# alibaba/euler

Hardware: AMD Instinct MI355X
Metric: sampled edges/sec (whole node), 2-hop fanout=[25,10], 100M-node power-law graph (higher is better)
Workload: dtype f64; 1 GPU; synthetic RMAT-marginal power-law graph, 100000000 nodes / 1000001082 edges (min degree 1), f32 weights uniform [0.5,8), weighted CDF-inversion SampleNeighbor, fanout [25,10], 131072 uniform-random roots per step per GPU, TF dense layout; graph_bytes_per_gpu=55296276736, partitioning=none, streams=3, repeats=1, full=False, ranks=1

## Files before the change

### euler_amd/_lib.py

```python
import ctypes as C
import os

HERE = os.path.dirname(os.path.abspath(__file__))
LIB_PATH = os.environ.get("EULER_GPU_LIB_PATH") or os.path.join(HERE, "lib", "libeuler_gpu.so")

OK, EINVAL, ENOMEM, EHIP, ENOGRAPH, EIO, EEMPTY = 0, -1, -2, -3, -4, -5, -6
LAYOUT_CORE, LAYOUT_TF = 0, 1
F32, BF16, F16 = 0, 1, 2

u64p = C.POINTER(C.c_uint64)
i64p = C.POINTER(C.c_int64)
i32p = C.POINTER(C.c_int32)
f32p = C.POINTER(C.c_float)
u8p = C.POINTER(C.c_uint8)
vp = C.c_void_p


class HostCSR(C.Structure):
    _fields_ = [("n_rows", C.c_int64), ("n_edge_types", C.c_int32),
                ("n_node_types", C.c_int32), ("row_id", u64p),
                ("row_ptr", i64p), ("type_end", i32p), ("nbr", u64p),
                ("prefix_w", f32p), ("type_prefix", f32p),
                ("node_type", i32p), ("node_weight", f32p),
                ("sampler_order", u64p),
# ... 70 lines not shown
    "euler_gpu_sample_graph_label": (C.c_int, [vp, vp, C.c_uint64, C.c_uint32, C.c_int32, vp]),
    "euler_gpu_get_graph_by_label": (C.c_int, [vp, vp, vp, C.c_int64, vp, i64p, vp]),
    "euler_gpu_whole_graph_block": (C.c_int, [vp, vp, vp, C.c_int64, i32p, C.c_int32, C.c_int32,
                                              C.c_int64, i64p, vp]),
    "euler_gpu_graph_destroy": (None, [vp]),
    "euler_gpu_graph_num_nodes": (C.c_int64, [vp]),
    "euler_gpu_graph_num_edges": (C.c_int64, [vp]),
    "euler_gpu_graph_num_edge_types": (C.c_int32, [vp]),
    "euler_gpu_graph_num_node_types": (C.c_int32, [vp]),
    "euler_gpu_graph_device": (C.c_int, [vp]),
    "euler_gpu_graph_bytes": (C.c_int64, [vp]),
    "euler_gpu_graph_node_weight_sums": (C.c_int, [vp, f32p]),
    "euler_gpu_graph_set_node_sampler": (C.c_int, [vp, C.c_int64, u64p, i32p, f32p, C.c_int32]),
    "euler_gpu_last_fanout_kernel": (C.c_char_p, []),
    "euler_gpu_graph_index_overflow_rows": (C.c_int, [vp, u64p, C.c_int64, i64p]),
    "euler_gpu_graph_export_rows": (C.c_int, [vp, u64p, C.c_int64, i64p, i32p, u64p,
                                              f32p, f32p]),
    "InitQueryProxy": (C.c_bool, [C.c_char_p]),
    "euler_gpu_default_graph": (vp, []),
    "euler_gpu_graph_partitions": (C.c_int32, [vp]),
    "euler_gpu_sample_neighbor": (C.c_int, [vp, vp, C.c_uint64, C.c_uint32, vp,
                                            C.c_int64, vp, C.c_int32, i32p, C.c_int32,
                                            C.c_int32, C.c_int32, C.c_int64, vp, vp,
                                            vp, vp]),
    "euler_gpu_sample_fanout_workspace": (C.c_size_t, [C.c_int64, i32p, C.c_int32]),
    "euler_gpu_sample_fanout": (C.c_int, [vp, vp, C.c_uint64, C.c_uint32, vp,
                                          C.c_int64, i32p, C.c_int32, i32p, C.c_int32,
                                          C.c_int64, C.POINTER(vp), C.POINTER(vp),
                                          C.POINTER(vp), vp]),
    "euler_gpu_sample_fanout_multi": (C.c_int, [vp, vp, C.c_uint64, C.c_uint32, C.c_uint32, vp,
# ... 257 lines not shown
```

### euler_amd/csrc/common.h

```cpp
#pragma once

#include <hip/hip_runtime.h>
#include <stdint.h>

#include <atomic>
#include <map>
#include <mutex>
#include <string>
#include <vector>

#include "../../include/euler_gpu.h"
#include "../../include/euler_gpu_measure.h"
#include "philox.h"

namespace euler_gpu {

void SetError(const std::string& msg);
int Fail(int code, const std::string& msg);

#define EG_HIP(expr)                                                        \
  do {                                                                      \
    hipError_t _e = (expr);                                                 \
    if (_e != hipSuccess)                                                   \
      return ::euler_gpu::Fail(EULER_GPU_EHIP,                              \
// ... 30 lines not shown
  const float* pivots;
  int64_t piv_off[kPivotLevels + 1];
  const float* bpiv;
  int64_t bpiv_off[kPivotLevels + 1];
  const struct EdgeBlock* blk;
  const float* skip1;
  int64_t n_blk;
  const struct WbRec* wrec;
  const struct EdgeBlock* wb;
  int64_t n_wb;
  const uint8_t* wbg;
  int32_t wbg_stride;
  const uint8_t* trec;
  int32_t trec_stride;
  const uint8_t* fat;
  int32_t wb_lean_ok;
};

inline bool HasBlockSearch(const GraphView& v) { return v.blk != nullptr || v.wbg != nullptr; }

constexpr int kEdgesPerBlock = 10;
struct alignas(128) EdgeBlock {
  float pw[kEdgesPerBlock];
  float prev_last;
  uint32_t pad;
  uint64_t nbr[kEdgesPerBlock];
};
static_assert(sizeof(EdgeBlock) == 128, "EdgeBlock must be one 128-byte line");

constexpr int kWavesPerSimd = 8;
// ... 84 lines not shown
  std::vector<std::pair<void*, int64_t>> edge_allocs;
  std::pair<void*, int64_t> edge_sampler_alloc{nullptr, 0};
  std::vector<int64_t> bin_host_ptr;
  std::vector<int32_t> bin_host_idx;
  std::vector<uint8_t> bin_host_val;
  int32_t bin_host_slots = 0;
  mutable std::mutex bin_mu;
  mutable euler_gpu::FeatTable node_bin{};
  mutable bool node_bin_ready = false;
  mutable std::mutex ws_mu;
  mutable std::recursive_mutex launch_mu;
  mutable std::map<void*, std::pair<void*, size_t>> ws;
  mutable std::map<void*, int> ws_parity;
  mutable std::atomic<void*> last_stream{nullptr};
  mutable std::atomic<int> wb_tried{0};
  std::vector<uint32_t> wb_overflow_rows;
  mutable std::atomic<int> blk_ready{0};
  struct FlowTableDense { void* p = nullptr; size_t rows = 0; uint32_t next_epoch = 1; };
  mutable std::map<void*, FlowTableDense> flow_tables;
  int32_t shards = 1;
  int32_t label_slot = -1;
  mutable std::mutex label_mu;
  mutable bool labels_ready = false;
  mutable int64_t n_labels = 0;
  mutable int64_t n_labelled = 0;
  mutable const uint64_t* label_nodes = nullptr;
  mutable const int64_t* label_start = nullptr;
  mutable std::vector<std::pair<void*, int64_t>> label_allocs;
  mutable std::vector<int64_t> label_off_host;
  mutable std::vector<uint8_t> label_bytes_host;
// ... 110 lines not shown
```

### euler_amd/csrc/fanout_local.h

```cpp
#ifndef EULER_AMD_CSRC_FANOUT_LOCAL_H_
#define EULER_AMD_CSRC_FANOUT_LOCAL_H_

#include <hip/hip_runtime.h>

#include "k1_search.h"
#include "wb_index.h"

namespace euler_gpu {

struct SmallDiv {
  uint32_t d, m;
  __host__ void Set(uint32_t div) { d = div; m = div <= 1 ? 0u : 0xFFFFFFFFu / div + 1u; }
  __device__ __forceinline__ uint32_t operator()(uint32_t n) const {
    return d <= 1 ? n : __umulhi(n, m);
  }
};

struct FanoutLocalArgs {
  GraphView g;
  uint64_t seed;
  const uint64_t* roots;
  int64_t n;
  int64_t default_node;
  uint32_t call_id;
// ... 510 lines not shown
  if (__ballot(cold0 || cold1) != 0ull) {
#pragma nounroll
    for (int s = 0; s < (TWO ? 2 : 1); ++s) {
      if (s == 0 ? cold0 : cold1) {
        const float* nw = g.prefix_w + rec.lo;
        const uint32_t mid = (uint32_t)RandomSelect(nw, 0, (uint64_t)(rec.deg - 1u), s == 0 ? u0 : u1);
        const uint64_t ci = g.nbr[rec.lo + mid];
        const float cw = __fsub_rn(nw[mid], mid == 0u ? 0.f : nw[mid - 1]);
        if (s == 0) { id[0] = ci; w[0] = cw; m[0] = rec.lo + mid; }
        else { id[1] = ci; w[1] = cw; m[1] = rec.lo + mid; }
      }
    }
  }
}

struct WbSeg {
  uint32_t wb_lo, row_deg;
  uint32_t lo, deg;
  float row_total, lim_b, lim_e;
  uint32_t row_lo;
};

__device__ __forceinline__ bool FatFind(const GraphView& g, const uint64_t id, uint4* hd, uint4* tl,
                                        const uint4** slot) {
  uint64_t h = Mix64(id) & g.hash_mask;
  for (uint64_t probes = 0; probes <= g.hash_mask; ++probes) {
    const uint4* s = reinterpret_cast<const uint4*>(g.fat + h * 64);
    const uint4 a = s[0], b = s[1];
    if ((int32_t)b.y == -1) return false;
    if (a.x == (uint32_t)id && a.y == (uint32_t)(id >> 32)) { *hd = a; *tl = b; *slot = s; return true; }
// ... 347 lines not shown
  L.o_mask = o; o += (uint32_t)gr * 8;
  L.o_sw = o; o += s * 4;
  L.o_w1 = o; o += p * 4;
  L.o_st = o; o += (uint32_t)cap * 4;
  L.o_slot = o; o += (p * 2 + 3) & ~3u;
  L.o_rvalid = o; o += ((uint32_t)gr + 3) & ~3u;
  L.o_t1 = o; L.o_t2 = o;
  if (typed) {
    o += (p + 3) & ~3u;
    L.o_t2 = o; o += (s + 3) & ~3u;
  }
  L.bytes = (o + 15) & ~15u;
  return L;
}

template <bool WIDE, int WPS, bool UNIFORM = false, int WB = 0>
__global__ __launch_bounds__(256, WPS) void SampleFanoutLeanKernel(
    const FanoutLocalArgs a) {
  extern __shared__ __align__(16) uint8_t fl_smem[];
  const int lane = threadIdx.x & 63;
  const int wave_in_block = __builtin_amdgcn_readfirstlane((int)(threadIdx.x >> 6));
  const int waves_per_block = blockDim.x >> 6;
  const FanoutLeanLds L = FanoutLeanLayout(a.gr, a.c1, a.c2, a.cap, WB >= 3 && WB <= 5);
  uint8_t* base = fl_smem + (size_t)wave_in_block * a.wave_lds;
  uint64_t* s_sid = reinterpret_cast<uint64_t*>(base + L.o_sid);
  uint64_t* s_c1 = reinterpret_cast<uint64_t*>(base + L.o_c1);
  uint64_t* s_slotid = reinterpret_cast<uint64_t*>(base + L.o_slotid);
  unsigned long long* s_mask = reinterpret_cast<unsigned long long*>(base + L.o_mask);
  float* s_sw = reinterpret_cast<float*>(base + L.o_sw);
  float* s_w1 = reinterpret_cast<float*>(base + L.o_w1);
  int32_t* s_st = reinterpret_cast<int32_t*>(base + L.o_st);
// ... 211 lines not shown
        const bool live = in && deg > 0 && !EG_FL_ABLATE(a, 2);
        uint64_t id[2]; float w[2]; uint32_t m[2];
        int32_t tt[2] = {a.t2, a.t2};
        bool sentinel = false;
        Philox4 pb;
        if (WB == 4 || WB == 5) WbSampleTypedPair4<WB == 5>(g, w4, a.type_mode, a.et2, a.k, a.seed, tile_call + 1u, node, xp, live,
                                        true, id, w, m, tt, &sentinel);
        else if (WB == 3) WbSampleTypedPair(g, wt, a.type_mode, a.et2, a.k, a.seed, tile_call + 1u, node, xp, live,
                                            true, id, w, m, tt, &sentinel);
        else pb = RngBlock(a.seed, tile_call + 1u, kDomainNeighbor, node, xp);
        if (WB >= 3 && WB <= 5) {}
        else if (WB == 6) UniformSamplePairG2(g, ws, ws, a.t2, a.t2, live, live, UnitFromWords(pb.w[0], pb.w[1]),
                                              UnitFromWords(pb.w[2], pb.w[3]), id, w, m);
        else if (WB == 2) WbSamplePairG(g, ws, a.t2, live, UnitFromWords(pb.w[0], pb.w[1]),
                                   UnitFromWords(pb.w[2], pb.w[3]), id, w, m);
        else if (WB) WbSamplePair(g, wr, live, UnitFromWords(pb.w[0], pb.w[1]),
                                  UnitFromWords(pb.w[2], pb.w[3]), id, w, m);
        else if (UNIFORM) LeanSamplePairUniform(g, lo, deg, total, live, UnitFromWords(pb.w[0], pb.w[1]),
                                           UnitFromWords(pb.w[2], pb.w[3]), id, w, m);
        else LeanSamplePair(g, lo, deg, total, live, UnitFromWords(pb.w[0], pb.w[1]),
                            UnitFromWords(pb.w[2], pb.w[3]), id, w, m, EG_FL_ABLATE_BITS(a));
        if (in) {
          fl_u64x2 iv;
          iv.x = live ? id[0] : (uint64_t)a.default_node;
          iv.y = live ? id[1] : (uint64_t)a.default_node;
          *reinterpret_cast<fl_u64x2*>(s_sid + sl * c2 + 2u * xp) = iv;
          *reinterpret_cast<float2*>(s_sw + sl * c2 + 2u * xp) =
              make_float2(live ? w[0] : 0.f, live ? w[1] : 0.f);
          if (xp == 0) s_st[sl] = live ? a.t2 : -1;
          if (WB >= 3 && WB <= 5) {
// ... 118 lines not shown
```

### euler_amd/csrc/fanout_plain.h

```cpp
#ifndef EULER_AMD_CSRC_FANOUT_PLAIN_H_
#define EULER_AMD_CSRC_FANOUT_PLAIN_H_

#include <hip/hip_runtime.h>

#include "fanout_local.h"

namespace euler_gpu {

struct FanoutPlainArgs {
  const WbRec* wrec;
  const EdgeBlock* wb;
  const float* prefix_w;
  const uint64_t* nbr;
  const uint64_t* roots;
  uint64_t* id1; float* w1; int32_t* ty1;
  uint64_t* id2; float* w2; int32_t* ty2;
  uint32_t* row_index;
  const uint32_t* call_ids;
  uint64_t seed, id_base, id_stride;
  int64_t n, n_rows, default_node, mb_n;
  uint32_t call_id, call_stride;
  int32_t c1, c2, gr, cap, wave_lds;
};

constexpr uint32_t kStageLines = 128;
constexpr uint32_t kStageBytes = kStageLines * 48 + kStageLines * 4;
// ... 247 lines not shown
__device__ __forceinline__ int64_t PlainFindRow(const FanoutPlainArgs& a, const uint64_t id) {
  const uint64_t d = id - a.id_base;
  if (id < a.id_base) return -1;
  if (a.id_stride == 1) return d < (uint64_t)a.n_rows ? (int64_t)d : -1;
  const uint64_t r = d / a.id_stride;
  return (r * a.id_stride == d && r < (uint64_t)a.n_rows) ? (int64_t)r : -1;
}

__device__ __forceinline__ WbRec PlainLoadRec(const FanoutPlainArgs& a, const uint64_t node) {
  WbRec wr{0u, 0u, 0u, 0.f};
  const int64_t row = PlainFindRow(a, node);
  if (row >= 0) wr = a.wrec[row];
  return wr;
}

template <int WPS, bool COOP, bool LITE2 = false>
__global__ __launch_bounds__(256, WPS) void SampleFanoutPlainKernel(const FanoutPlainArgs a) {
  extern __shared__ __align__(16) uint8_t fp_smem[];
  const uint32_t lane = threadIdx.x & 63u;
  const int wave_in_block = __builtin_amdgcn_readfirstlane((int)(threadIdx.x >> 6));
  const int waves_per_block = blockDim.x >> 6;
  const uint32_t c1 = (uint32_t)a.c1, c2 = (uint32_t)a.c2, gr = (uint32_t)a.gr, cap = (uint32_t)a.cap;
  const FanoutPlainLds L = FanoutPlainLayout(a.gr, a.c1, a.c2, a.cap, COOP);
  uint8_t* base = fp_smem + (size_t)wave_in_block * a.wave_lds;
  float4* s_stage = reinterpret_cast<float4*>(base + L.o_stage);
  uint32_t* s_blk = reinterpret_cast<uint32_t*>(base + L.o_blk);
  uint64_t* s_sid = reinterpret_cast<uint64_t*>(base + L.o_sid);
  uint64_t* s_c1 = reinterpret_cast<uint64_t*>(base + L.o_c1);
  unsigned long long* s_mask = reinterpret_cast<unsigned long long*>(base + L.o_mask);
  float* s_sw = reinterpret_cast<float*>(base + L.o_sw);
  float* s_w1 = reinterpret_cast<float*>(base + L.o_w1);
// ... 120 lines not shown
      const uint32_t rs = d_hp2(lane2), x2 = lane2 - __umul24(rs, hp2);
      const bool act2 = rs < RPI;
      for (uint32_t sb = 0; sb < ns; sb += RPI) {
        const uint32_t sl = sb + rs;
        const bool in = act2 && sl < ns;
        uint64_t child = 0;
        WbRec cr{0u, 0u, 0u, 0.f};
        if (in) { child = s_c1[s_rep[s0 + sl]]; cr = PlainLoadRec(a, child); }
        const bool lv = in && cr.deg > 0u;
        uint64_t i2[2]; float w2[2]; uint32_t m2[2];
        const Philox4 pb = RngBlock(a.seed, call + 1u, kDomainNeighbor, child, x2);
        if (COOP) {
          const uint32_t left = ns - sb < RPI ? ns - sb : RPI;
          WaveSamplePairs(a, lane, __umul24(left, hp2), s_stage, s_blk, cr, lv, lv, UnitFromWords(pb.w[0], pb.w[1]),
                          UnitFromWords(pb.w[2], pb.w[3]), i2, w2, m2);
        } else if (LITE2) {
          PlainSamplePairLite(a, cr, lv, lv, UnitFromWords(pb.w[0], pb.w[1]), UnitFromWords(pb.w[2], pb.w[3]), i2, w2);
        } else {
          PlainSamplePair(a, cr, lv, lv, UnitFromWords(pb.w[0], pb.w[1]), UnitFromWords(pb.w[2], pb.w[3]),
                          i2, w2, m2);
        }
        if (in) {
          fl_u64x2 iv;
          iv.x = lv ? i2[0] : (uint64_t)a.default_node;
          iv.y = lv ? i2[1] : (uint64_t)a.default_node;
          const uint32_t at = __umul24(sl, c2) + 2u * x2;
          *reinterpret_cast<fl_u64x2*>(s_sid + at) = iv;
          *reinterpret_cast<float2*>(s_sw + at) = make_float2(lv ? w2[0] : 0.f, lv ? w2[1] : 0.f);
          if (x2 == 0) s_st[sl] = lv ? 0 : -1;
        }
// ... 104 lines not shown
```

### euler_amd/csrc/graph_build.hip

```cpp
#include <hip/hip_runtime.h>
#include <sys/stat.h>
#include <hipcub/hipcub.hpp>

#include <algorithm>
#include <atomic>
#include <cstdlib>
#include <cmath>
#include <cstring>
#include <map>
#include <memory>
#include <mutex>
#include <sstream>

#include "device_fns.h"
#include "device_mem.h"
#include "wb_index.h"

namespace euler_gpu {


namespace {
thread_local std::string g_last_error;
std::mutex g_default_mu;
euler_gpu_graph* g_default_graph = nullptr;
}

void SetError(const std::string& msg) { g_last_error = msg; }
int Fail(int code, const std::string& msg) {
  g_last_error = msg;
  return code;
}
// ... 773 lines not shown
    }
    const RowMeta m = LoadRowMeta(g, lo);
    const uint32_t deg = (uint32_t)m.type_end[g.T - 1];
    EdgeBlock e;
    if (WbBuildBlock(g.prefix_w, g.nbr, (uint32_t)m.row_ptr, deg, g.prefix_w[m.row_ptr + deg - 1],
                     (uint32_t)(b - (int64_t)wb_lo[lo]), &e)) {
      ++mine;
      const unsigned long long k = atomicAdd(overflows + 1, 1ull);
      if (k < (unsigned long long)kWbOverflowKeep) ovf_rows[k] = (uint32_t)lo;
    }
    wb[b] = e;
  }
  if (mine != 0) atomicAdd(overflows, mine);
}

__global__ __launch_bounds__(256) void FatFillKernel(GraphView g, const uint8_t* trec, int32_t trec_stride,
                                                     uint8_t* fat) {
  const uint64_t stride = (uint64_t)gridDim.x * blockDim.x;
  for (uint64_t h = (uint64_t)blockIdx.x * blockDim.x + threadIdx.x; h <= g.hash_mask; h += stride) {
    const uint64_t key = g.hash_slots[2 * h];
    const int64_t row = (int64_t)g.hash_slots[2 * h + 1];
    uint4 a = make_uint4(0u, 0u, 0u, 0u), b = make_uint4(0u, 0xFFFFFFFFu, 0u, 0u), c = make_uint4(0u, 0u, 0u, 0u);
    if (row >= 0) {
      const uint8_t* rec = trec + row * (int64_t)trec_stride;
      const uint32_t* hd = reinterpret_cast<const uint32_t*>(rec);
      const int32_t* te = reinterpret_cast<const int32_t*>(rec + 8);
      const float* lim = reinterpret_cast<const float*>(rec + 8 + 4 * g.T);
      const RowMeta m = LoadRowMeta(g, row);
      const int32_t t1 = g.T - 1;
      a = make_uint4((uint32_t)key, (uint32_t)(key >> 32), hd[0], hd[1]);
// ... 41 lines not shown
    if (f >= 0 && f <= 1) ppm = (int64_t)(f * 1e6);
  }
  g_wb_budget_ppm.store(ppm);
  g_wb_budget_bytes.store(bytes);
}

bool WbFits(size_t need) {
  WbBudgetFromEnv();
  size_t free_b = 0, total_b = 0;
  if (hipMemGetInfo(&free_b, &total_b) != hipSuccess) { (void)hipGetLastError(); return false; }
  const int64_t cap = g_wb_budget_bytes.load();
  if (cap >= 0 && need > (size_t)cap) return false;
  const double frac = (double)g_wb_budget_ppm.load() * 1e-6;
  if ((double)need > frac * (double)free_b) return false;
  return need + ((size_t)1 << 30) <= free_b;
}

int BuildWbIndex(GraphBuilder* b) {
  GraphView& v = b->g->view;
  if (v.monotone != 0 && v.uniform_w != 0 && (v.T > 1 || v.map_mode != 0) && v.n_rows > 0 && v.n_edges > 0 &&
      v.n_edges < ((int64_t)1 << 31)) {
    const int32_t stride = v.T == 1 ? 16 : 8 + 12 * v.T;
    if (!WbFits((size_t)v.n_rows * stride)) return EULER_GPU_OK;
    uint8_t* trec = b->Alloc<uint8_t>((size_t)v.n_rows * stride + 16);
    if (b->rc != EULER_GPU_OK) return b->rc;
    hipLaunchKernelGGL(WbRecKernel, dim3((v.n_rows + 255) / 256), dim3(256), 0, 0, v, (const uint32_t*)nullptr,
                       trec, stride);
    EG_HIP(hipGetLastError());
    EG_HIP(hipDeviceSynchronize());
    v.trec = trec; v.trec_stride = stride;
// ... 39 lines not shown
  EG_HIP(hipMemset(ovf, 0, 16 + 4 * kWbOverflowKeep));
  if (n_wb > 0)
    hipLaunchKernelGGL(WbFillKernel, dim3(GridFor(n_wb, block)), dim3(block), 0, 0, v, wb_lo, n_wb, wb, ovf);
  EG_HIP(hipGetLastError());
  EG_HIP(hipDeviceSynchronize());
  unsigned long long n_ovf = 0;
  EG_HIP(hipMemcpy(&n_ovf, ovf, 8, hipMemcpyDeviceToHost));
  {
    const size_t keep = (size_t)std::min<unsigned long long>(n_ovf, (unsigned long long)kWbOverflowKeep);
    b->g->wb_overflow_rows.resize(keep);
    if (keep > 0) EG_HIP(hipMemcpy(b->g->wb_overflow_rows.data(), ovf + 2, keep * 4, hipMemcpyDeviceToHost));
  }
  v.wrec = rec; v.wb = wb; v.n_wb = n_wb; v.wbg = wbg; v.wbg_stride = stride;
  v.trec = wbg; v.trec_stride = stride;
  v.wb_lean_ok = (double)n_ovf <= 0.002 * (double)n_wb ? 1 : 0;
  return BuildFatSlots(b);
}

int EnsureWbIndex(const euler_gpu_graph* cg) {
  euler_gpu_graph* g = const_cast<euler_gpu_graph*>(cg);
  if (g->wb_tried.load(std::memory_order_acquire) != 0) return EULER_GPU_OK;
  std::lock_guard<std::mutex> lk(g_blocked_mu);
  if (g->wb_tried.load(std::memory_order_acquire) != 0) return EULER_GPU_OK;
  DeviceGuard dg(g->device);
  GraphBuilder b;
  b.g.reset(g);
  const int rc = BuildWbIndex(&b);
  if (rc == EULER_GPU_OK) b.Commit();
  b.g.release();
  if (rc != EULER_GPU_OK) {
    (void)hipGetLastError();
    (void)hipDeviceSynchronize();
    (void)hipGetLastError();
    b.Release();
    GraphView& v = g->view;
    v.wb = nullptr; v.wbg = nullptr; v.wrec = nullptr; v.n_wb = 0; v.wb_lean_ok = 0;
    v.trec = nullptr; v.trec_stride = 0; v.fat = nullptr;
  }
  g->wb_tried.store(1, std::memory_order_release);
  return EULER_GPU_OK;
}

std::atomic<int> g_blk_fail_next{0};

int EnsureBlockedIndex(const euler_gpu_graph* cg) {
  euler_gpu_graph* g = const_cast<euler_gpu_graph*>(cg);
  if (g->blk_ready.load(std::memory_order_acquire) != 0) return EULER_GPU_OK;
  std::lock_guard<std::mutex> lk(g_blocked_mu);
  if (g->blk_ready.load(std::memory_order_acquire) != 0) return EULER_GPU_OK;
  DeviceGuard dg(g->device);
  GraphBuilder b;
  b.g.reset(g);
// ... 235 lines not shown
int euler_gpu_graph_index_overflow_rows(const euler_gpu_graph* g, uint64_t* ids_host, int64_t cap,
                                        int64_t* n_host) {
  if (!g || !n_host || cap < 0 || (cap > 0 && !ids_host))
    return Fail(EULER_GPU_EINVAL, "index_overflow_rows: bad arguments");
  *n_host = 0;
  const int rc = EnsureWbIndex(g);
  if (rc != EULER_GPU_OK) return rc;
  const GraphView& v = g->view;
  if (v.map_mode != 0) return EULER_GPU_OK;
  int64_t n = 0;
  for (uint32_t row : g->wb_overflow_rows) {
    if (n >= cap) break;
    ids_host[n++] = v.id_base + v.id_stride * (uint64_t)row;
  }
  *n_host = n;
  return EULER_GPU_OK;
}

int euler_gpu_graph_node_weight_sums(const euler_gpu_graph* g, float* out_host) {
  if (!g || !out_host) return Fail(EULER_GPU_EINVAL, "node_weight_sums: null");
  for (size_t i = 0; i < g->node_weight_sums.size(); ++i)
    out_host[i] = g->node_weight_sums[i];
  return EULER_GPU_OK;
}

int euler_gpu_graph_export_rows(const euler_gpu_graph* g, const uint64_t* ids_host,
                                int64_t n, int64_t* row_ptr_host,
                                int32_t* type_end_host, uint64_t* nbr_host,
                                float* prefix_w_host, float* type_prefix_host) {
  if (!g) return Fail(EULER_GPU_ENOGRAPH, "export_rows: null graph");
// ... 104 lines not shown
```

### euler_amd/csrc/sample_kernels.hip

```cpp
#include <hip/hip_runtime.h>
#include <hipcub/hipcub.hpp>

#include <cmath>
#include <vector>

#include "device_mem.h"
#include "k1_args.h"
#include "k1_search.h"
#include "fanout_local.h"
#include "fanout_plain.h"

extern thread_local int g_feature_vec4;
namespace euler_gpu { extern thread_local int g_walk_collapse, g_walk_grid, g_walk_tail, g_walk_lean; extern std::atomic<int> g_walk_path_ch, g_n2v_list_big, g_n2v_list_big_parent, g_n2v_list_merged, g_n2v_walk_tickets; }
namespace euler_gpu { extern std::atomic<int> g_sharded_self_exchange, g_sharded_walk_enqueued, g_sharded_walk_tail, g_sharded_walk_split; }
namespace euler_gpu { extern std::atomic<int> g_flow_fused; extern std::atomic<int> g_flow_rowpos; }
namespace euler_gpu { extern std::atomic<int> g_blk_fail_next; }
namespace euler_gpu { extern thread_local int g_label_hash_bits; }
namespace euler_gpu { extern thread_local int g_root_host_batch, g_adj_scan, g_adj_long_row, g_sum_scalar; }

namespace euler_gpu {

struct DedupArgs {
  GraphView g;
  const uint64_t* roots;
// ... 445 lines not shown
thread_local int g_fanout_fused = 1;
thread_local int g_full_nb_balanced = 1;
thread_local int g_n2v_big = 8192;
thread_local int g_fanout_local = 1;
thread_local int g_fl_roots = 0;
thread_local int g_fl_cap = 0;
thread_local int g_fl_block = 0;
thread_local int g_fl_wide = 1;
thread_local int g_fl_grid_cap = -1;
thread_local int g_fl_min_roots = 32768;
thread_local int g_fl_plain = 2;
thread_local int g_fl_wps = 5;
thread_local int g_fp_on = 1;
thread_local int g_fp_coop = 0;
thread_local int g_fp_lite2 = 0;
thread_local int g_fp_wps = 5;
thread_local int g_fl_wb = 1;
thread_local int g_fl_typed_regs = 1;
thread_local int g_k1_sets_lds = 1;
thread_local int g_fl_fat = 1;
thread_local int g_blk_policy = 0;
thread_local int g_fl_ablate = 0;
thread_local int g_k1_typed_pivot = 1;
thread_local uint32_t* t_fl_row_index = nullptr;
thread_local int t_fl_took_lean = 0;
thread_local const char* t_fl_last_kernel = "";
thread_local void* g_fl_debug = nullptr;

int SamplingView(const euler_gpu_graph* g, GraphView* out) {
  const bool wb = g_fl_wb != 0 && g_k1_variant == 6;
  if (wb) {
    const int rc = EnsureWbIndex(g);
    if (rc != EULER_GPU_OK) return rc;
  }
  const bool wb_serves = wb && g->view.wbg != nullptr && (g->view.wb_lean_ok != 0 || g_blk_policy == 1);
  if (g_k1_variant == 6 && !wb_serves && g->blk_ready.load(std::memory_order_acquire) == 0) {
    const int rc = EnsureBlockedIndex(g);
    if (rc != EULER_GPU_OK) return rc;
  }
  *out = g->view;
  if (!wb) { out->wb = nullptr; out->wbg = nullptr; out->wrec = nullptr; out->n_wb = 0; out->wb_lean_ok = 0;
             out->trec = nullptr; out->trec_stride = 0; out->fat = nullptr; }
  if (g_fl_fat == 0) out->fat = nullptr;
  return EULER_GPU_OK;
}

template <bool TF_LAYOUT, int U, bool BLOCKED>
__device__ __forceinline__ void PivotPass(const SampleNbArgs& a, const int64_t n_roots,
                                          const int64_t stride_rows,
                                          const int32_t stride_slots) {
  const int64_t total = n_roots * (int64_t)a.count;
  const int64_t stride = (int64_t)gridDim.x * blockDim.x * U;
  int64_t s = ((int64_t)blockIdx.x * blockDim.x + threadIdx.x) * U;
  if (s >= total) return;
  int64_t r = s / a.count;
  int32_t j = (int32_t)(s - r * a.count);
  const int32_t t = a.et[0];
// ... 784 lines not shown
          ll = FanoutLeanLayout(gr, c1, c2, lcap, lean_t);
        }
        const bool use_wb0 = v.uniform_w == 0 && f.g.wrec != nullptr && f.g.wb != nullptr && v.wb_lean_ok != 0;
        if (g_fp_on != 0 && (t_concurrent != 1 || g_fp_on == 2 || big) && plain && !typed_hops && use_wb0 && f.wide) {
          int32_t pgr = g_fl_roots > 0 ? gr : 4;
          while (multi != nullptr && pgr > 1 && multi->n_per % pgr != 0) pgr >>= 1;
          int32_t pcap = g_fl_cap > 0 ? g_fl_cap : (g_fp_coop != 0 ? 64 / (c2 / 2 > 0 ? c2 / 2 : 1) : 32);
          if (pcap > pgr * c1) pcap = pgr * c1;
          const int pblock = (g_fl_block == 64 || g_fl_block == 128 || g_fl_block == 256) ? g_fl_block : 128;
          const bool coop = g_fp_coop != 0;
          const FanoutPlainLds pl = FanoutPlainLayout(pgr, c1, c2, pcap, coop);
          const int64_t tp = (int64_t)pgr * c1 * c2;
          if (pgr * ((c1 + 1) / 2) <= 64 && pgr * c1 <= 255 && pgr * c1 % 4 == 0 && tp % 4 == 0 && c2 <= 64 &&
              c1 <= 128 && (int64_t)pcap * c2 < 4096 && (size_t)pl.bytes * (pblock / 64) <= 64 * 1024) {
            FanoutPlainArgs pa{};
            pa.wrec = f.g.wrec; pa.wb = f.g.wb; pa.prefix_w = f.g.prefix_w; pa.nbr = f.g.nbr;
            pa.roots = roots_dev;
            pa.id1 = f.id1; pa.w1 = f.w1; pa.ty1 = f.ty1; pa.id2 = f.id2; pa.w2 = f.w2; pa.ty2 = f.ty2;
            pa.row_index = t_fl_row_index;
            pa.call_ids = f.call_ids; pa.seed = seed; pa.id_base = f.g.id_base; pa.id_stride = f.g.id_stride;
            pa.n = n; pa.n_rows = f.g.n_rows; pa.default_node = default_node; pa.mb_n = f.mb_n;
            pa.call_id = call_id; pa.call_stride = f.call_stride;
            pa.c1 = c1; pa.c2 = c2; pa.gr = pgr; pa.cap = pcap; pa.wave_lds = (int32_t)pl.bytes;
            const int64_t ptiles = (n + pgr - 1) / pgr;
            const int pwpb = pblock / 64;
            int64_t pblocks = (ptiles + pwpb - 1) / pwpb;
            int64_t pwaves = g_fl_grid_cap > 0 ? g_fl_grid_cap : 0;
            if (pwaves > 0 && pblocks > (pwaves + pwpb - 1) / pwpb) pblocks = (pwaves + pwpb - 1) / pwpb;
            void (*pk)(const FanoutPlainArgs) = nullptr;
#define EG_FP(W) (coop ? SampleFanoutPlainKernel<W, true, false> : g_fp_lite2 != 0 ? SampleFanoutPlainKernel<W, false, true> \
                       : SampleFanoutPlainKernel<W, false, false>)
            pk = g_fp_wps >= 8 ? EG_FP(8) : g_fp_wps == 7 ? EG_FP(7) : g_fp_wps == 6 ? EG_FP(6)
                 : g_fp_wps == 5 ? EG_FP(5) : EG_FP(4);
#undef EG_FP
            t_fl_took_lean = 1;
            t_fl_last_kernel = "SampleFanoutPlainKernel";
            hipLaunchKernelGGL(pk, dim3((unsigned)pblocks), dim3(pblock), (size_t)pl.bytes * pwpb, stream, pa);
            EG_HIP(hipGetLastError());
            if (uniq_off != nullptr) { uniq_off[0] = -1; uniq_off[1] = -1; }
            return EULER_GPU_OK;
          }
        }
        if (!big && (size_t)ll.bytes * (block / 64) <= 64 * 1024) {
          f.cap = lcap; f.wave_lds = (int32_t)ll.bytes;
          f.div_h1.Set((uint32_t)(c1 + 1) / 2); f.div_h2.Set((uint32_t)c2 / 2);
          const size_t llds = (size_t)ll.bytes * wpb;
// ... 7 lines not shown
          const bool use_wb = v.uniform_w == 0 && f.g.wrec != nullptr && f.g.wb != nullptr && v.wb_lean_ok != 0;
          if (lean_gu) {
            lk = f.wide ? SampleFanoutLeanKernel<true, 5, false, 6> : SampleFanoutLeanKernel<false, 5, false, 6>;
          } else if (lean_tu) {
            lk = f.wide ? SampleFanoutLeanKernel<true, 5, false, 5> : SampleFanoutLeanKernel<false, 5, false, 5>;
          } else if (lean_t && v.T <= 4 && g_fl_typed_regs != 0) {
            lk = f.wide ? SampleFanoutLeanKernel<true, 5, false, 4> : SampleFanoutLeanKernel<false, 5, false, 4>;
          } else if (lean_t) {
            lk = f.wide ? SampleFanoutLeanKernel<true, 5, false, 3> : SampleFanoutLeanKernel<false, 5, false, 3>;
          } else if (lean_g) {
            lk = f.wide ? (g_fl_wps == 6 ? SampleFanoutLeanKernel<true, 6, false, 2> : SampleFanoutLeanKernel<true, 5, false, 2>)
                        : (g_fl_wps == 6 ? SampleFanoutLeanKernel<false, 6, false, 2> : SampleFanoutLeanKernel<false, 5, false, 2>);
          } else if (v.uniform_w != 0) {
            lk = g_fl_wps == 8 ? (f.wide ? SampleFanoutLeanKernel<true, 8, true> : SampleFanoutLeanKernel<false, 8, true>)
                               : (f.wide ? SampleFanoutLeanKernel<true, 5, true> : SampleFanoutLeanKernel<false, 5, true>);
          } else if (use_wb) {
            lk = f.wide ? (g_fl_wps == 8 ? SampleFanoutLeanKernel<true, 8, false, 1>
                                         : g_fl_wps == 5 ? SampleFanoutLeanKernel<true, 5, false, 1>
                                                         : SampleFanoutLeanKernel<true, 6, false, 1>)
                        : (g_fl_wps == 8 ? SampleFanoutLeanKernel<false, 8, false, 1>
                                         : g_fl_wps == 5 ? SampleFanoutLeanKernel<false, 5, false, 1>
                                                         : SampleFanoutLeanKernel<false, 6, false, 1>);
          } else {
            lk = f.wide ? (g_fl_wps == 8 ? SampleFanoutLeanKernel<true, 8>
                                         : g_fl_wps == 5 ? SampleFanoutLeanKernel<true, 5>
                                                         : SampleFanoutLeanKernel<true, 6>)
                        : (g_fl_wps == 8 ? SampleFanoutLeanKernel<false, 8>
                                         : g_fl_wps == 5 ? SampleFanoutLeanKernel<false, 5>
                                                         : SampleFanoutLeanKernel<false, 6>);
          }
// ... 215 lines not shown
  if (key == 52 && (value == 0 || value == 1)) { g_sharded_self_exchange.store(value); return EULER_GPU_OK; }
  if (key == 53 && value >= 0 && value <= 2) { g_fp_on = value; return EULER_GPU_OK; }
  if (key == 54 && (value == 0 || value == 1)) { g_fp_coop = value; return EULER_GPU_OK; }
  if (key == 57 && (value == 0 || value == 1)) { g_fp_lite2 = value; return EULER_GPU_OK; }
  if (key == 60 && (value == 0 || value == 1)) { g_flow_fused.store(value); return EULER_GPU_OK; }
  if (key == 62 && value >= 0 && value <= 2) { g_flow_rowpos.store(value); return EULER_GPU_OK; }
  if (key == 69 && value >= 0) { g_n2v_list_big.store(value); return EULER_GPU_OK; }
  if (key == 71 && value >= 0) { g_n2v_list_big_parent.store(value); return EULER_GPU_OK; }
  if (key == 72 && (value == 0 || value == 1)) { g_n2v_list_merged.store(value); return EULER_GPU_OK; }
  if (key == 73 && (value == 0 || value == 1)) { g_n2v_walk_tickets.store(value); return EULER_GPU_OK; }
  if (key == 67 && value >= 0 && value <= 1024) { g_sharded_walk_split.store(value); return EULER_GPU_OK; }
  if (key == 66 && value >= 0 && value <= 1024) { g_sharded_walk_tail.store(value); return EULER_GPU_OK; }
  if (key == 64 && value >= 1 && value <= 64) { g_walk_path_ch.store(value); return EULER_GPU_OK; }
  if (key == 63 && (value == 0 || value == 1)) { g_sharded_walk_enqueued.store(value); return EULER_GPU_OK; }
  if (key == 55 && value >= 4 && value <= 8) { g_fp_wps = value; return EULER_GPU_OK; }
  if (key == 56 && value >= 0) { g_blk_fail_next.store(value); return EULER_GPU_OK; }
  return Fail(EULER_GPU_EINVAL, "set_tuning: unknown key");
}

const char* euler_gpu_last_fanout_kernel(void) { return t_fl_last_kernel; }

int euler_gpu_sample_fanout_multi(const euler_gpu_graph* g, void* stream, uint64_t seed,
                                  uint32_t call_id, uint32_t call_stride,
                                  const uint32_t* call_ids_dev, int32_t m,
                                  const uint64_t* roots_dev, int64_t n,
                                  const int32_t* edge_types_host, int32_t k,
                                  const int32_t* counts_host, int32_t layers,
                                  int64_t default_node, uint64_t* const* out_id_dev,
                                  float* const* out_w_dev, int32_t* const* out_t_dev,
                                  void* workspace_dev) {
// ... 548 lines not shown
```

### euler_amd/graph.py

```python
import contextlib
import ctypes as C
import math
import threading

import numpy as np
import torch

from . import _lib
from ._lib import check, lib

_I32 = C.POINTER(C.c_int32)


_RAW_STREAM = getattr(torch._C, "_cuda_getCurrentRawStream", None)


def _stream():
    if _RAW_STREAM is not None:
        return C.c_void_p(_RAW_STREAM(torch.cuda.current_device()))
    return C.c_void_p(torch.cuda.current_stream().cuda_stream)


def _ptr(t):
    return C.c_void_p(t.data_ptr()) if t is not None else None
# ... 302 lines not shown
        check(lib().euler_gpu_graph_export_rows(
            self._h, ids.ctypes.data_as(_lib.u64p), n,
            row_ptr.ctypes.data_as(_lib.i64p), None, None, None, None))
        tot = int(row_ptr[-1])
        type_end = np.zeros(n * T, np.int32)
        nbr = np.zeros(max(tot, 1), np.uint64)
        pw = np.zeros(max(tot, 1), np.float32)
        tp = np.zeros(n * T, np.float32)
        check(lib().euler_gpu_graph_export_rows(
            self._h, ids.ctypes.data_as(_lib.u64p), n,
            row_ptr.ctypes.data_as(_lib.i64p), type_end.ctypes.data_as(_lib.i32p),
            nbr.ctypes.data_as(_lib.u64p), pw.ctypes.data_as(_lib.f32p),
            tp.ctypes.data_as(_lib.f32p)))
        return row_ptr, type_end, nbr[:tot], pw[:tot], tp

    def index_overflow_rows(self, cap=4096):
        out = np.zeros(max(int(cap), 1), np.uint64)
        n = C.c_int64(0)
        check(lib().euler_gpu_graph_index_overflow_rows(self._h, out.ctypes.data_as(_lib.u64p), int(cap),
                                                        C.byref(n)))
        return out[:n.value]


    def _on_device(self):
        if torch.cuda.current_device() == self._dev_index:
            return _NULL_CTX
        return torch.cuda.device(self.device)

    def set_seed(self, seed, call_id=0):
        with self._lock:
# ... 975 lines not shown
```

### include/euler_gpu_measure.h

```cpp
#ifndef EULER_GPU_MEASURE_H_
#define EULER_GPU_MEASURE_H_

#include "euler_gpu.h"

#ifdef __cplusplus
extern "C" {
#endif

int euler_gpu_set_tuning(int32_t key, int32_t value);
int euler_gpu_set_debug_buffer(void* dev);

const char* euler_gpu_last_fanout_kernel(void);

int euler_gpu_graph_index_overflow_rows(const euler_gpu_graph* g, uint64_t* ids_host, int64_t cap,
                                        int64_t* n_host);

int euler_gpu_time_sample_neighbor(const euler_gpu_graph* g, void* stream,
                                   uint64_t seed, const uint64_t* roots_dev,
                                   int64_t n, const int32_t* edge_types_host,
                                   int32_t k, int32_t count, int32_t layout,
                                   uint64_t* out_id_dev, float* out_w_dev,
                                   int32_t* out_t_dev, int32_t iters,
                                   float* mean_ms_host);
int euler_gpu_time_sample_neighbor_phases(const euler_gpu_graph* g, void* stream,
                                          uint64_t seed, const uint64_t* roots_dev,
                                          int64_t n, const int32_t* edge_types_host,
                                          int32_t k, int32_t count, int32_t layout,
                                          int32_t dedup, uint64_t* out_id_dev,
                                          float* out_w_dev, int32_t* out_t_dev,
                                          int32_t iters, float* mean_ms3_host,
// ... 37 lines not shown
```

Before: 167.2 billion sampled edges/s.

## Add header-plus-window side index for hop-2 weighted neighbor sampling

Builds a second per-bucket 128-byte line (HwLine) for each weight-bucket block. Each line holds a quantized 8-entry prefix header and 9 interleaved (id, prefix-weight) entries, so a draw can guess its slot from the header and then read one small window instead of scanning a whole EdgeBlock. The plain and lean fanout kernels gain an HW template path that is on by default. Draws that miss the window fall back to binary search over prefix_w. This costs extra device memory (one more line per bucket, gated by the index budget) and a build-time fill kernel, and the path is declined if more than 2 in 1000 lines overflow.

```diff
diff --git a/euler_amd/_lib.py b/euler_amd/_lib.py
--- a/euler_amd/_lib.py
+++ b/euler_amd/_lib.py
@@ -108,6 +108,7 @@
     "euler_gpu_graph_set_node_sampler": (C.c_int, [vp, C.c_int64, u64p, i32p, f32p, C.c_int32]),
     "euler_gpu_last_fanout_kernel": (C.c_char_p, []),
     "euler_gpu_graph_index_overflow_rows": (C.c_int, [vp, u64p, C.c_int64, i64p]),
+    "euler_gpu_graph_side_index": (C.c_int, [vp, i64p, i64p, i64p]),
     "euler_gpu_graph_export_rows": (C.c_int, [vp, u64p, C.c_int64, i64p, i32p, u64p,
                                               f32p, f32p]),
     "InitQueryProxy": (C.c_bool, [C.c_char_p]),
diff --git a/euler_amd/csrc/common.h b/euler_amd/csrc/common.h
--- a/euler_amd/csrc/common.h
+++ b/euler_amd/csrc/common.h
@@ -68,6 +68,7 @@
   const uint8_t* trec;
   int32_t trec_stride;
   const uint8_t* fat;
+  const struct HwLine* hw;
   int32_t wb_lean_ok;
 };
 
@@ -182,6 +183,7 @@
   mutable std::map<void*, int> ws_parity;
   mutable std::atomic<void*> last_stream{nullptr};
   mutable std::atomic<int> wb_tried{0};
+  int64_t hw_bytes = 0, hw_lines = 0, hw_overflows = 0;
   std::vector<uint32_t> wb_overflow_rows;
   mutable std::atomic<int> blk_ready{0};
   struct FlowTableDense { void* p = nullptr; size_t rows = 0; uint32_t next_epoch = 1; };
diff --git a/euler_amd/csrc/fanout_local.h b/euler_amd/csrc/fanout_local.h
--- a/euler_amd/csrc/fanout_local.h
+++ b/euler_amd/csrc/fanout_local.h
@@ -5,6 +5,7 @@
 
 #include "k1_search.h"
 #include "wb_index.h"
+#include "wb_hw.h"
 
 namespace euler_gpu {
 
@@ -548,6 +549,46 @@
   }
 }
 
+__device__ __forceinline__ void HwSamplePair(const HwLine* hw, const float* prefix_w, const uint64_t* nbr,
+                                             const WbRec rec, const bool live, const double u0,
+                                             const double u1, uint64_t id[2], float w[2]) {
+  const double r0 = __dmul_rn(u0, (double)rec.total), r1 = __dmul_rn(u1, (double)rec.total);
+  const bool t0 = live && (double)rec.total > r0, t1 = live && (double)rec.total > r1;
+  const float f0 = WbFloorToFloat(r0), f1 = WbFloorToFloat(r1);
+  const uint32_t nbk = WbBuckets(rec.deg);
+  uint32_t j0 = 0u, j1 = 0u;
+  if (nbk > 1u) {
+    const float scale = WbScale(nbk, rec.total);
+    j0 = WbBucketOf(f0, nbk, scale);
+    j1 = WbBucketOf(f1, nbk, scale);
+  }
+  const HwLine* l0 = hw + rec.wb_lo + j0;
+  const HwLine* l1 = hw + rec.wb_lo + j1;
+  const HwHead h0 = HwLoadHead(l0), h1 = HwLoadHead(l1);
+  const uint32_t i0 = HwGuess(h0, f0), i1 = HwGuess(h1, f1);
+  const HwPre p0 = HwLoadPre(l0, i0), p1 = HwLoadPre(l1, i1);
+  const HwWin x0 = HwLoadWin(l0, i0), x1 = HwLoadWin(l1, i1);
+  id[0] = 0; id[1] = 0; w[0] = 0.f; w[1] = 0.f;
+  const int32_t d0 = HwPick(p0, x0, i0, f0, &id[0], &w[0]), d1 = HwPick(p1, x1, i1, f1, &id[1], &w[1]);
+  const bool hot0 = t0 && d0 == 0, hot1 = t1 && d1 == 0;
+  if (!hot0) { id[0] = 0; w[0] = 0.f; }
+  if (!hot1) { id[1] = 0; w[1] = 0.f; }
+  const bool cold0 = live && !hot0, cold1 = live && !hot1;
+  if (__ballot(cold0 || cold1) != 0ull) {
+#pragma nounroll
+    for (int s = 0; s < 2; ++s) {
+      if (s == 0 ? cold0 : cold1) {
+        const float* nw = prefix_w + rec.lo;
+        const uint32_t mid = (uint32_t)RandomSelect(nw, 0, (uint64_t)(rec.deg - 1u), s == 0 ? u0 : u1);
+        const uint64_t ci = nbr[rec.lo + mid];
+        const float cw = __fsub_rn(nw[mid], mid == 0u ? 0.f : nw[mid - 1]);
+        if (s == 0) { id[0] = ci; w[0] = cw; }
+        else { id[1] = ci; w[1] = cw; }
+      }
+    }
+  }
+}
+
 struct WbSeg {
   uint32_t wb_lo, row_deg;
   uint32_t lo, deg;
@@ -925,7 +966,7 @@
   return L;
 }
 
-template <bool WIDE, int WPS, bool UNIFORM = false, int WB = 0>
+template <bool WIDE, int WPS, bool UNIFORM = false, int WB = 0, bool HW = false>
 __global__ __launch_bounds__(256, WPS) void SampleFanoutLeanKernel(
     const FanoutLocalArgs a) {
   extern __shared__ __align__(16) uint8_t fl_smem[];
@@ -1167,6 +1208,8 @@
                                               UnitFromWords(pb.w[2], pb.w[3]), id, w, m);
         else if (WB == 2) WbSamplePairG(g, ws, a.t2, live, UnitFromWords(pb.w[0], pb.w[1]),
                                    UnitFromWords(pb.w[2], pb.w[3]), id, w, m);
+        else if (WB == 1 && HW) HwSamplePair(g.hw, g.prefix_w, g.nbr, wr, live, UnitFromWords(pb.w[0], pb.w[1]),
+                                             UnitFromWords(pb.w[2], pb.w[3]), id, w);
         else if (WB) WbSamplePair(g, wr, live, UnitFromWords(pb.w[0], pb.w[1]),
                                   UnitFromWords(pb.w[2], pb.w[3]), id, w, m);
         else if (UNIFORM) LeanSamplePairUniform(g, lo, deg, total, live, UnitFromWords(pb.w[0], pb.w[1]),
diff --git a/euler_amd/csrc/fanout_plain.h b/euler_amd/csrc/fanout_plain.h
--- a/euler_amd/csrc/fanout_plain.h
+++ b/euler_amd/csrc/fanout_plain.h
@@ -10,6 +10,7 @@
 struct FanoutPlainArgs {
   const WbRec* wrec;
   const EdgeBlock* wb;
+  const HwLine* hw;
   const float* prefix_w;
   const uint64_t* nbr;
   const uint64_t* roots;
@@ -287,7 +288,7 @@
   return wr;
 }
 
-template <int WPS, bool COOP, bool LITE2 = false>
+template <int WPS, bool COOP, bool LITE2 = false, bool HW = false>
 __global__ __launch_bounds__(256, WPS) void SampleFanoutPlainKernel(const FanoutPlainArgs a) {
   extern __shared__ __align__(16) uint8_t fp_smem[];
   const uint32_t lane = threadIdx.x & 63u;
@@ -438,6 +439,9 @@
           const uint32_t left = ns - sb < RPI ? ns - sb : RPI;
           WaveSamplePairs(a, lane, __umul24(left, hp2), s_stage, s_blk, cr, lv, lv, UnitFromWords(pb.w[0], pb.w[1]),
                           UnitFromWords(pb.w[2], pb.w[3]), i2, w2, m2);
+        } else if (HW) {
+          HwSamplePair(a.hw, a.prefix_w, a.nbr, cr, lv, UnitFromWords(pb.w[0], pb.w[1]),
+                       UnitFromWords(pb.w[2], pb.w[3]), i2, w2);
         } else if (LITE2) {
           PlainSamplePairLite(a, cr, lv, lv, UnitFromWords(pb.w[0], pb.w[1]), UnitFromWords(pb.w[2], pb.w[3]), i2, w2);
         } else {
diff --git a/euler_amd/csrc/graph_build.hip b/euler_amd/csrc/graph_build.hip
--- a/euler_amd/csrc/graph_build.hip
+++ b/euler_amd/csrc/graph_build.hip
@@ -15,6 +15,7 @@
 #include "device_fns.h"
 #include "device_mem.h"
 #include "wb_index.h"
+#include "wb_hw.h"
 
 namespace euler_gpu {
 
@@ -818,6 +819,27 @@
   if (mine != 0) atomicAdd(overflows, mine);
 }
 
+__global__ __launch_bounds__(256) void HwFillKernel(GraphView g, const uint32_t* wb_lo, int64_t n_wb,
+                                                    HwLine* hw, unsigned long long* overflows) {
+  const int64_t stride = (int64_t)gridDim.x * blockDim.x;
+  unsigned long long mine = 0;
+  for (int64_t b = (int64_t)blockIdx.x * blockDim.x + threadIdx.x; b < n_wb; b += stride) {
+    int64_t lo = 0, hi = g.n_rows;
+    while (hi - lo > 1) {
+      const int64_t mid = (lo + hi) >> 1;
+      if ((int64_t)wb_lo[mid] <= b) lo = mid; else hi = mid;
+    }
+    const RowMeta m = LoadRowMeta(g, lo);
+    const uint32_t deg = (uint32_t)m.type_end[g.T - 1];
+    HwLine e;
+    if (HwBuildLine(g.prefix_w, g.nbr, (uint32_t)m.row_ptr, deg, g.prefix_w[m.row_ptr + deg - 1],
+                    (uint32_t)(b - (int64_t)wb_lo[lo]), &e))
+      ++mine;
+    hw[b] = e;
+  }
+  if (mine != 0) atomicAdd(overflows, mine);
+}
+
 __global__ __launch_bounds__(256) void FatFillKernel(GraphView g, const uint8_t* trec, int32_t trec_stride,
                                                      uint8_t* fat) {
   const uint64_t stride = (uint64_t)gridDim.x * blockDim.x;
@@ -889,6 +911,47 @@
   const double frac = (double)g_wb_budget_ppm.load() * 1e-6;
   if ((double)need > frac * (double)free_b) return false;
   return need + ((size_t)1 << 30) <= free_b;
+}
+
+void BuildHwSide(GraphBuilder* b, const uint32_t* wb_lo, int64_t n_wb) {
+  static std::atomic<int> said{0};
+  GraphView& v = b->g->view;
+  auto decline = [&](const char* why) {
+    (void)hipGetLastError();
+    if (said.exchange(1) == 0)
+      fprintf(stderr, "euler_gpu: header + window side index declined (%s); hop 2 of the fanout step keeps "
+                      "the weight-bucket blocks\n", why);
+  };
+  const size_t bytes = (size_t)n_wb * sizeof(HwLine);
+  if (!WbFits(bytes)) { decline("over the index budget"); return; }
+  DevBuf cnt;
+  AllocList side("");
+  HwLine* hw = side.Alloc<HwLine>((size_t)n_wb);
+  if (hw == nullptr || cnt.alloc(16) != hipSuccess || hipMemset(cnt.as(), 0, 16) != hipSuccess) {
+    side.Release();
+    decline("no memory");
+    return;
+  }
+  hipLaunchKernelGGL(HwFillKernel, dim3(GridFor(n_wb, 256)), dim3(256), 0, 0, v, wb_lo, n_wb, hw,
+                     cnt.as<unsigned long long>());
+  unsigned long long n_ovf = 0;
+  if (hipGetLastError() != hipSuccess || hipDeviceSynchronize() != hipSuccess ||
+      hipMemcpy(&n_ovf, cnt.as(), 8, hipMemcpyDeviceToHost) != hipSuccess) {
+    side.Release();
+    decline("build failed");
+    return;
+  }
+  if ((double)n_ovf > 0.002 * (double)n_wb) {
+    side.Release();
+    decline("more than 2 lines in a thousand overflow");
+    return;
+  }
+  for (auto& blk : side.list) b->list.push_back(blk);
+  side.list.clear();
+  v.hw = hw;
+  b->g->hw_bytes = (int64_t)std::max<size_t>(bytes, 16);
+  b->g->hw_lines = n_wb;
+  b->g->hw_overflows = (int64_t)n_ovf;
 }
 
 int BuildWbIndex(GraphBuilder* b) {
@@ -958,6 +1021,7 @@
   v.wrec = rec; v.wb = wb; v.n_wb = n_wb; v.wbg = wbg; v.wbg_stride = stride;
   v.trec = wbg; v.trec_stride = stride;
   v.wb_lean_ok = (double)n_ovf <= 0.002 * (double)n_wb ? 1 : 0;
+  if (plain && v.has_zero_nbr == 0 && v.wb_lean_ok != 0 && n_wb > 0) BuildHwSide(b, wb_lo, n_wb);
   return BuildFatSlots(b);
 }
 
@@ -980,6 +1044,7 @@
     GraphView& v = g->view;
     v.wb = nullptr; v.wbg = nullptr; v.wrec = nullptr; v.n_wb = 0; v.wb_lean_ok = 0;
     v.trec = nullptr; v.trec_stride = 0; v.fat = nullptr;
+    v.hw = nullptr; g->hw_bytes = 0; g->hw_lines = 0; g->hw_overflows = 0;
   }
   g->wb_tried.store(1, std::memory_order_release);
   return EULER_GPU_OK;
@@ -1245,6 +1310,16 @@
     ids_host[n++] = v.id_base + v.id_stride * (uint64_t)row;
   }
   *n_host = n;
+  return EULER_GPU_OK;
+}
+
+int euler_gpu_graph_side_index(const euler_gpu_graph* g, int64_t* bytes_host, int64_t* lines_host,
+                               int64_t* overflows_host) {
+  if (!g || !bytes_host || !lines_host || !overflows_host)
+    return Fail(EULER_GPU_EINVAL, "graph_side_index: null argument");
+  const int rc = EnsureWbIndex(g);
+  if (rc != EULER_GPU_OK) return rc;
+  *bytes_host = g->hw_bytes; *lines_host = g->hw_lines; *overflows_host = g->hw_overflows;
   return EULER_GPU_OK;
 }
 
diff --git a/euler_amd/csrc/sample_kernels.hip b/euler_amd/csrc/sample_kernels.hip
--- a/euler_amd/csrc/sample_kernels.hip
+++ b/euler_amd/csrc/sample_kernels.hip
@@ -483,6 +483,7 @@
 thread_local int g_fp_on = 1;
 thread_local int g_fp_coop = 0;
 thread_local int g_fp_lite2 = 0;
+thread_local int g_fp_hw = 1;
 thread_local int g_fp_wps = 5;
 thread_local int g_fl_wb = 1;
 thread_local int g_fl_typed_regs = 1;
@@ -509,7 +510,7 @@
   }
   *out = g->view;
   if (!wb) { out->wb = nullptr; out->wbg = nullptr; out->wrec = nullptr; out->n_wb = 0; out->wb_lean_ok = 0;
-             out->trec = nullptr; out->trec_stride = 0; out->fat = nullptr; }
+             out->hw = nullptr; out->trec = nullptr; out->trec_stride = 0; out->fat = nullptr; }
   if (g_fl_fat == 0) out->fat = nullptr;
   return EULER_GPU_OK;
 }
@@ -1324,7 +1325,8 @@
           if (pgr * ((c1 + 1) / 2) <= 64 && pgr * c1 <= 255 && pgr * c1 % 4 == 0 && tp % 4 == 0 && c2 <= 64 &&
               c1 <= 128 && (int64_t)pcap * c2 < 4096 && (size_t)pl.bytes * (pblock / 64) <= 64 * 1024) {
             FanoutPlainArgs pa{};
-            pa.wrec = f.g.wrec; pa.wb = f.g.wb; pa.prefix_w = f.g.prefix_w; pa.nbr = f.g.nbr;
+            const bool hw2 = g_fp_hw != 0 && f.g.hw != nullptr && !coop && g_fp_lite2 == 0;
+            pa.wrec = f.g.wrec; pa.wb = f.g.wb; pa.hw = f.g.hw; pa.prefix_w = f.g.prefix_w; pa.nbr = f.g.nbr;
             pa.roots = roots_dev;
             pa.id1 = f.id1; pa.w1 = f.w1; pa.ty1 = f.ty1; pa.id2 = f.id2; pa.w2 = f.w2; pa.ty2 = f.ty2;
             pa.row_index = t_fl_row_index;
@@ -1339,7 +1341,7 @@
             if (pwaves > 0 && pblocks > (pwaves + pwpb - 1) / pwpb) pblocks = (pwaves + pwpb - 1) / pwpb;
             void (*pk)(const FanoutPlainArgs) = nullptr;
 #define EG_FP(W) (coop ? SampleFanoutPlainKernel<W, true, false> : g_fp_lite2 != 0 ? SampleFanoutPlainKernel<W, false, true> \
-                       : SampleFanoutPlainKernel<W, false, false>)
+                       : hw2 ? SampleFanoutPlainKernel<W, false, false, true> : SampleFanoutPlainKernel<W, false, false>)
             pk = g_fp_wps >= 8 ? EG_FP(8) : g_fp_wps == 7 ? EG_FP(7) : g_fp_wps == 6 ? EG_FP(6)
                  : g_fp_wps == 5 ? EG_FP(5) : EG_FP(4);
 #undef EG_FP
@@ -1377,6 +1379,13 @@
           } else if (v.uniform_w != 0) {
             lk = g_fl_wps == 8 ? (f.wide ? SampleFanoutLeanKernel<true, 8, true> : SampleFanoutLeanKernel<false, 8, true>)
                                : (f.wide ? SampleFanoutLeanKernel<true, 5, true> : SampleFanoutLeanKernel<false, 5, true>);
+          } else if (use_wb && plain && g_fp_hw != 0 && f.g.hw != nullptr) {
+            lk = f.wide ? (g_fl_wps == 8 ? SampleFanoutLeanKernel<true, 8, false, 1, true>
+                                         : g_fl_wps == 5 ? SampleFanoutLeanKernel<true, 5, false, 1, true>
+                                                         : SampleFanoutLeanKernel<true, 6, false, 1, true>)
+                        : (g_fl_wps == 8 ? SampleFanoutLeanKernel<false, 8, false, 1, true>
+                                         : g_fl_wps == 5 ? SampleFanoutLeanKernel<false, 5, false, 1, true>
+                                                         : SampleFanoutLeanKernel<false, 6, false, 1, true>);
           } else if (use_wb) {
             lk = f.wide ? (g_fl_wps == 8 ? SampleFanoutLeanKernel<true, 8, false, 1>
                                          : g_fl_wps == 5 ? SampleFanoutLeanKernel<true, 5, false, 1>
@@ -1622,6 +1631,7 @@
   if (key == 64 && value >= 1 && value <= 64) { g_walk_path_ch.store(value); return EULER_GPU_OK; }
   if (key == 63 && (value == 0 || value == 1)) { g_sharded_walk_enqueued.store(value); return EULER_GPU_OK; }
   if (key == 55 && value >= 4 && value <= 8) { g_fp_wps = value; return EULER_GPU_OK; }
+  if (key == 75 && (value == 0 || value == 1)) { g_fp_hw = value; return EULER_GPU_OK; }
   if (key == 56 && value >= 0) { g_blk_fail_next.store(value); return EULER_GPU_OK; }
   return Fail(EULER_GPU_EINVAL, "set_tuning: unknown key");
 }
diff --git a/euler_amd/csrc/wb_hw.h b/euler_amd/csrc/wb_hw.h
--- /dev/null
+++ b/euler_amd/csrc/wb_hw.h
@@ -0,0 +1,127 @@
+#ifndef EULER_AMD_CSRC_WB_HW_H_
+#define EULER_AMD_CSRC_WB_HW_H_
+
+#include "wb_index.h"
+
+namespace euler_gpu {
+
+constexpr uint32_t kHwEntries = 9;
+constexpr uint32_t kHwQMax = 254;
+
+struct alignas(128) HwLine { uint32_t w[32]; };
+static_assert(sizeof(HwLine) == 128, "HwLine must be one 128-byte line");
+
+struct alignas(16) HwHead { uint32_t invq, q0, q1, base; };
+struct __attribute__((packed, aligned(4))) HwWin { uint32_t before, id_lo, id_hi, sum; };
+
+EG_HD float HwAsFloat(uint32_t x) { return __builtin_bit_cast(float, x); }
+EG_HD uint32_t HwAsBits(float x) { return __builtin_bit_cast(uint32_t, x); }
+
+EG_HD bool HwBuildLine(const float* prefix_w, const uint64_t* nbr, uint32_t lo, uint32_t deg,
+                       float total, uint32_t j, HwLine* out) {
+  const uint32_t nbk = WbBuckets(deg);
+  const ArraySum nw{prefix_w + lo};
+  const float scale = WbScale(nbk, total);
+  const uint32_t s = WbBlockStart(nw, deg, nbk, scale, j);
+  bool overflow = false;
+  if (s + kHwEntries < deg) {
+    if (j + 1u >= nbk) {
+      overflow = true;
+    } else {
+      const double U = ((double)(j + 1u) / (double)scale) * (1.0 + 1.0 / 1048576.0);
+      overflow = !((double)nw(s + kHwEntries - 1u) > U);
+    }
+  }
+  const float base = s == 0u ? 0.f : prefix_w[lo + s - 1u];
+  const uint32_t nreal = deg - s < 8u ? deg - s : 8u;
+  const float range = EG_FSUB(prefix_w[lo + s + nreal - 1u], base);
+  float invq = EG_FDIV((float)kHwQMax, range);
+  if (!(invq > 0.f) || !(invq < __builtin_huge_valf())) invq = 0.f;
+  uint32_t q[2] = {0u, 0u};
+  for (uint32_t k = 0; k < 8u; ++k) {
+    uint32_t v = 255u;
+    if (s + k < deg) {
+      const float t = EG_FMUL(EG_FSUB(prefix_w[lo + s + k], base), invq);
+      v = !(t >= 0.f) ? 0u : (t < (float)kHwQMax ? (uint32_t)t : kHwQMax);
+    }
+    q[k >> 2] |= v << (8u * (k & 3u));
+  }
+  out->w[0] = HwAsBits(invq); out->w[1] = q[0]; out->w[2] = q[1]; out->w[3] = HwAsBits(base);
+  for (uint32_t k = 0; k < kHwEntries; ++k) {
+    const uint32_t m = s + k;
+    const bool in = m < deg;
+    const uint64_t id = in ? nbr[lo + m] : 0ull;
+    out->w[4u + 3u * k] = (uint32_t)id;
+    out->w[5u + 3u * k] = (uint32_t)(id >> 32);
+    out->w[6u + 3u * k] = HwAsBits(in ? prefix_w[lo + m] : __builtin_huge_valf());
+  }
+  out->w[31] = lo + s;
+  return overflow;
+}
+
+EG_HD HwHead HwLoadHead(const HwLine* ln) { return *reinterpret_cast<const HwHead*>(ln->w); }
+
+struct __attribute__((packed, aligned(4))) HwPre { uint32_t before, id_lo, id_hi; };
+EG_HD HwPre HwLoadPre(const HwLine* ln, uint32_t i) {
+  return *reinterpret_cast<const HwPre*>(ln->w + 3u * i);
+}
+
+EG_HD HwWin HwLoadWin(const HwLine* ln, uint32_t i) {
+  return *reinterpret_cast<const HwWin*>(ln->w + 3u + 3u * i);
+}
+
+EG_HD uint32_t HwGuess(const HwHead& h, float f) {
+  const float t = EG_FMUL(EG_FSUB(f, HwAsFloat(h.base)), HwAsFloat(h.invq));
+  const uint32_t ti = !(t >= 0.f) ? 0u : (t < (float)kHwQMax ? (uint32_t)t : kHwQMax);
+  uint32_t i = 0;
+  i += ((h.q0) & 255u) <= ti ? 1u : 0u;
+  i += ((h.q0 >> 8) & 255u) <= ti ? 1u : 0u;
+  i += ((h.q0 >> 16) & 255u) <= ti ? 1u : 0u;
+  i += (h.q0 >> 24) <= ti ? 1u : 0u;
+  i += ((h.q1) & 255u) <= ti ? 1u : 0u;
+  i += ((h.q1 >> 8) & 255u) <= ti ? 1u : 0u;
+  i += ((h.q1 >> 16) & 255u) <= ti ? 1u : 0u;
+  i += (h.q1 >> 24) <= ti ? 1u : 0u;
+  return i;
+}
+
+EG_HD int32_t HwCheck(const HwWin& x, float f, uint64_t* id, float* w) {
+  const float before = HwAsFloat(x.before), sum = HwAsFloat(x.sum);
+  const int32_t d = before > f ? -1 : (!(sum > f) ? 1 : 0);
+  *id = d == 0 ? ((uint64_t)x.id_lo | ((uint64_t)x.id_hi << 32)) : *id;
+  *w = d == 0 ? EG_FSUB(sum, before) : *w;
+  return d;
+}
+
+EG_HD int32_t HwPick(const HwPre& pre, const HwWin& win, uint32_t i, float f, uint64_t* id, float* w) {
+  const int32_t d = HwCheck(win, f, id, w);
+  const bool prev = d < 0 && i != 0u && !(HwAsFloat(pre.before) > f);
+  *id = prev ? ((uint64_t)pre.id_lo | ((uint64_t)pre.id_hi << 32)) : *id;
+  *w = prev ? EG_FSUB(HwAsFloat(win.before), HwAsFloat(pre.before)) : *w;
+  return prev ? 0 : d;
+}
+
+EG_HD int32_t HwDraw(const HwLine* ln, float f, uint64_t* id, float* w) {
+  const uint32_t i = HwGuess(HwLoadHead(ln), f);
+  const HwWin win = HwLoadWin(ln, i);
+  const int32_t d = HwCheck(win, f, id, w);
+  if (d == 0) return 1;
+  return HwPick(HwLoadPre(ln, i), win, i, f, id, w) == 0 ? 2 : -1;
+}
+
+EG_HD bool HwSampleHot(const HwLine* hw, const WbRec& rec, double u, uint64_t* id, float* w,
+                       int32_t* windows) {
+  const double r = EG_DMUL(u, (double)rec.total);
+  *windows = 0;
+  if (!((double)rec.total > r)) return false;
+  const float f = WbFloorToFloat(r);
+  const uint32_t nbk = WbBuckets(rec.deg);
+  const uint32_t j = nbk <= 1u ? 0u : WbBucketOf(f, nbk, WbScale(nbk, rec.total));
+  const int32_t n = HwDraw(hw + rec.wb_lo + j, f, id, w);
+  *windows = n < 0 ? 2 : n;
+  return n > 0;
+}
+
+}
+
+#endif
diff --git a/euler_amd/graph.py b/euler_amd/graph.py
--- a/euler_amd/graph.py
+++ b/euler_amd/graph.py
@@ -340,6 +340,11 @@
             tp.ctypes.data_as(_lib.f32p)))
         return row_ptr, type_end, nbr[:tot], pw[:tot], tp
 
+    def side_index(self):
+        b, n, o = C.c_int64(0), C.c_int64(0), C.c_int64(0)
+        check(lib().euler_gpu_graph_side_index(self._h, C.byref(b), C.byref(n), C.byref(o)))
+        return b.value, n.value, o.value
+
     def index_overflow_rows(self, cap=4096):
         out = np.zeros(max(int(cap), 1), np.uint64)
         n = C.c_int64(0)
diff --git a/include/euler_gpu_measure.h b/include/euler_gpu_measure.h
--- a/include/euler_gpu_measure.h
+++ b/include/euler_gpu_measure.h
@@ -14,6 +14,9 @@
 
 int euler_gpu_graph_index_overflow_rows(const euler_gpu_graph* g, uint64_t* ids_host, int64_t cap,
                                         int64_t* n_host);
+
+int euler_gpu_graph_side_index(const euler_gpu_graph* g, int64_t* bytes_host, int64_t* lines_host,
+                               int64_t* overflows_host);
 
 int euler_gpu_time_sample_neighbor(const euler_gpu_graph* g, void* stream,
                                    uint64_t seed, const uint64_t* roots_dev,
```

Result: faster. 185.3 billion sampled edges/s (median of 6 runs) (+10.8%).
